# jipolanco/PencilArrays.jl

Measured on NVIDIA H100. Metric: transpose_GiB_per_s, higher is better.
Workload: dtype c128 (bytes; pure data movement)

## Files before the change

### pencilarrays.jl_b200/csrc/fft.cu

```cuda
#include <cuda_runtime.h>

#include <algorithm>
#include <cmath>
#include <map>
#include <mutex>
#include <tuple>
#include <type_traits>
#include <vector>

#ifndef PA_FFT_TWIDDLE_LOOKUPS
#define PA_FFT_TWIDDLE_LOOKUPS 1
#endif
#include "fft_core.hpp"
#include "flags.cuh"
#include "pa_internal.hpp"

namespace pa {

using pa_fft::cplx;
using pa_fft::cplx_t;

template <class T>
struct Vec2;
template <>
struct Vec2<double> {
  using type = double2;
};
template <>
struct Vec2<float> {
  using type = float2;
};
__device__ __forceinline__ double2 vec2(double x, double y) { return make_double2(x, y); }
__device__ __forceinline__ float2 vec2(float x, float y) { return make_float2(x, y); }

template <class T, int STRIDE = 1>
struct Twiddles {
  const typename Vec2<T>::type* tab;
  __device__ __forceinline__ cplx_t<T> operator()(int k) const {
    const typename Vec2<T>::type w = __ldg(tab + STRIDE * k);
    return cplx_t<T>{w.x, w.y};
  }
};

constexpr int FFT_MAXB = 8;
constexpr int FFT_MAXO = PA_MAX_DIMS - 2;
constexpr int FFT_THREADS = 256;
constexpr int fft_lines(int logL) { return logL >= 10 ? 4 : 8; }
constexpr int fft_lines_f32(int logL) { return logL >= 10 ? 8 : 16; }

struct FftBlock {
  const char* src;
  int y0, ey;
  long long ssy;
  long long ssx;
  long long so[FFT_MAXO];
};
struct FftParams {
  int nb;
  FftBlock blk[FFT_MAXB];
  char* dst;
  long long ex;
  long long dsx;
  int no;
  long long oe[FFT_MAXO], dso[FFT_MAXO];
  int L, logL, sign, pitch;
  int linear;
  const void* tw;
  unsigned tiles_x;
  const void* tw4;
  int sine;
};

template <class T>
struct SmLine {
  cplx_t<T>* p;
  __device__ __forceinline__ cplx_t<T> get(int i) const { return p[pa_fft::pad_index(i)]; }
  __device__ __forceinline__ void put(int i, cplx_t<T> v) { p[pa_fft::pad_index(i)] = v; }
};

template <int LOGM>
struct PassRadix {
  static constexpr int LOGR = (LOGM % 3 == 0) ? 3 : (LOGM % 3);
};

template <int LOGL, int LOGM, int C, class T, class Tw>
__device__ __forceinline__ void fft_passes(cplx_t<T>* sm, int pitch, int ncol, int sign, const Tw& tw) {
  if constexpr (LOGM > 0) {
    constexpr int LOGR = PassRadix<LOGM>::LOGR;
    constexpr int R = 1 << LOGR, L = 1 << LOGL, M = 1 << LOGM;
    constexpr int PER_LINE = L / R;
    constexpr int TOTAL = C * PER_LINE;
#pragma unroll
    for (int w0 = 0; w0 < TOTAL; w0 += FFT_THREADS) {
      const int w = w0 + (int)threadIdx.x;
      const int c = w / PER_LINE, u = w % PER_LINE;
      if (w < TOTAL && c < ncol) {
        SmLine<T> x{sm + c * pitch};
        pa_fft::butterfly<R>(x, u, L, M, sign, tw);
      }
    }
    __syncthreads();
    fft_passes<LOGL, LOGM - LOGR, C>(sm, pitch, ncol, sign, tw);
  }
}

template <int LOGL, int LOGM>
__device__ __forceinline__ int fft_pos(int k) {
  if constexpr (LOGM == 0) {
    return 0;
  } else {
    constexpr int LOGR = PassRadix<LOGM>::LOGR;
    return ((k & ((1 << LOGR) - 1)) << (LOGM - LOGR)) + fft_pos<LOGL, LOGM - LOGR>(k >> LOGR);
  }
}

template <int LOGL, class T>
__device__ __forceinline__ T out_real(const T* line, int i) {
  return line[2 * pa_fft::pad_index(fft_pos<LOGL, LOGL>(i >> 1)) + (i & 1)];
}

template <int C, class T>
__device__ __forceinline__ void gather_rows(const FftParams& p, const long long* so_off, long long x0,
                                            int c, int r, int ncol, cplx_t<T>* line) {
  using V = typename Vec2<T>::type;
  constexpr int RS = FFT_THREADS / C;
  constexpr int U = 8;
#pragma unroll
  for (int b = 0; b < FFT_MAXB; ++b) {
    if (b < p.nb) {
      const FftBlock& B = p.blk[b];
      const char* s = B.src + so_off[b] + (x0 + c) * B.ssx;
      const int ey = B.ey, y0 = B.y0;
      const long long ssy = B.ssy;
      for (int y = r; y < ey; y += U * RS) {
        V v[U];
#pragma unroll
        for (int k = 0; k < U; ++k) {
          const int yy = y + k * RS;
          if (c < ncol && yy < ey) v[k] = __ldcs(reinterpret_cast<const V*>(s + (long long)yy * ssy));
        }
#pragma unroll
        for (int k = 0; k < U; ++k) {
          const int yy = y + k * RS;
          if (c < ncol && yy < ey) line[pa_fft::pad_index(y0 + yy)] = cplx_t<T>{v[k].x, v[k].y};
        }
      }
    }
  }
}

enum class RealMap {
  rfft,
  dct2,
  dct3,
};

template <RealMap MAP, int LOGL, class T>
__device__ __forceinline__ void put_real(T* line, int n, T x, bool sine) {
  constexpr int L = 1 << LOGL, N = 2 * L;
  if constexpr (MAP == RealMap::rfft) {
    line[2 * pa_fft::pad_index(n >> 1) + (n & 1)] = x;
  } else if constexpr (MAP == RealMap::dct2) {
    const int i = (n & 1) ? N - 1 - (n >> 1) : (n >> 1);
    line[2 * pa_fft::pad_index(i >> 1) + (i & 1)] = ((n & 1) && sine) ? -x : x;
  } else {
    const int j = sine ? N - 1 - n : n;
    if (j <= L) line[2 * pa_fft::pad_index(j)] = x;
    if (j >= L) line[2 * pa_fft::pad_index(N - j) + 1] = x;
  }
}

template <int C, class T, class Put>
__device__ __forceinline__ void gather_real_rows(const FftParams& p, const long long* so_off, long long x0,
                                                 int c, int r, int ncol, const Put& put) {
  constexpr int RS = FFT_THREADS / C;
  constexpr int U = 8;
#pragma unroll
  for (int b = 0; b < FFT_MAXB; ++b) {
    if (b < p.nb) {
      const FftBlock& B = p.blk[b];
      const char* s = B.src + so_off[b] + (x0 + c) * B.ssx;
      const int ey = B.ey, y0 = B.y0;
      const long long ssy = B.ssy;
      for (int y = r; y < ey; y += U * RS) {
        T v[U];
#pragma unroll
        for (int k = 0; k < U; ++k) {
          const int yy = y + k * RS;
          if (c < ncol && yy < ey) v[k] = __ldcs(reinterpret_cast<const T*>(s + (long long)yy * ssy));
        }
#pragma unroll
        for (int k = 0; k < U; ++k) {
          const int yy = y + k * RS;
          if (c < ncol && yy < ey) put(y0 + yy, v[k]);
        }
      }
    }
  }
}

__device__ __forceinline__ long long cta_offsets(const FftParams& p, int C, long long* so_off,
                                                 long long* d_off) {
  unsigned long long bid = blockIdx.x;
  const long long x0 = (long long)(bid % p.tiles_x) * C;
  bid /= p.tiles_x;
#pragma unroll
  for (int b = 0; b < FFT_MAXB; ++b) so_off[b] = 0;
  *d_off = 0;
#pragma unroll 1
  for (int i = 0; i < p.no; ++i) {
    const long long k = (long long)(bid % (unsigned long long)p.oe[i]);
    bid /= (unsigned long long)p.oe[i];
    *d_off += k * p.dso[i];
#pragma unroll
    for (int b = 0; b < FFT_MAXB; ++b)
      if (b < p.nb) so_off[b] += k * p.blk[b].so[i];
  }
  return x0;
}

template <int LOGL, int C, class T>
struct FftCtaShape {
  static constexpr int RS = FFT_THREADS / C;
  static constexpr int LOGRS = (C == 16) ? 4 : (C == 8) ? 5 : 6;
  static_assert((1 << LOGRS) == RS, "rows per sweep");
  static constexpr int LOGR1 = (sizeof(T) == 8 && C == 4 && LOGL > LOGRS) ? (LOGL - LOGRS) : 0;
  static_assert(LOGR1 == 0 || LOGL - LOGR1 == LOGRS, "first-pass stride must equal the sweep");
  static_assert(LOGR1 <= 4, "the register first pass is at most radix 16");
};

template <int LOGL, int C, class T>
__device__ __forceinline__ void fft_cta_lines(const FftParams& p, const long long* so_off, long long x0,
                                              int ncol, cplx_t<T>* sm) {
  using cx = cplx_t<T>;
  using V = typename Vec2<T>::type;
  constexpr int L = 1 << LOGL;
  const int t = threadIdx.x;
  const int pitch = p.pitch;

  constexpr int RS = FftCtaShape<LOGL, C, T>::RS;
  constexpr int LOGR1 = FftCtaShape<LOGL, C, T>::LOGR1;
  const V* twp = reinterpret_cast<const V*>(p.tw);
  const Twiddles<T> tw{twp};
  {
    const int c = p.linear ? t / RS : t % C, r = p.linear ? t % RS : t / C;
    cx* line = sm + c * pitch;
    if constexpr (LOGR1 > 0) {
      constexpr int R1 = 1 << LOGR1;
      if (c < ncol) {
        V v[R1];
#pragma unroll
        for (int q = 0; q < R1; ++q) {
          const int y = r + q * RS;
          const char* s = nullptr;
#pragma unroll
          for (int b = 0; b < FFT_MAXB; ++b)
            if (b < p.nb && y >= p.blk[b].y0 && y < p.blk[b].y0 + p.blk[b].ey)
              s = p.blk[b].src + so_off[b] + (long long)(y - p.blk[b].y0) * p.blk[b].ssy +
                  (x0 + c) * p.blk[b].ssx;
          v[q] = __ldcs(reinterpret_cast<const V*>(s));
        }
        cx a[R1];
#pragma unroll
        for (int q = 0; q < R1; ++q) a[q] = cx{v[q].x, v[q].y};
        pa_fft::butterfly_regs<R1>(a, r, L, L, p.sign, tw);
#pragma unroll
        for (int q = 0; q < R1; ++q) line[pa_fft::pad_index(r + q * RS)] = a[q];
      }
    } else {
      gather_rows<C, T>(p, so_off, x0, c, r, ncol, line);
    }
  }
  __syncthreads();

  fft_passes<LOGL, LOGL - LOGR1, C>(sm, pitch, ncol, p.sign, tw);
}

template <int LOGL, int LOGR1>
__device__ __forceinline__ int fft_out_pos(int k) {
  return ((k & ((1 << LOGR1) - 1)) << (LOGL - LOGR1)) + fft_pos<LOGL, LOGL - LOGR1>(k >> LOGR1);
}

template <int LOGL, int C, class T>
__device__ __forceinline__ void unpack_fft_cta(const FftParams& p) {
  using cx = cplx_t<T>;
  using V = typename Vec2<T>::type;
  constexpr int L = 1 << LOGL;
  extern __shared__ __align__(16) unsigned char fft_smem[];
  cx* sm = reinterpret_cast<cx*>(fft_smem);
  const int t = threadIdx.x;
  long long so_off[FFT_MAXB], d_off;
  const long long x0 = cta_offsets(p, C, so_off, &d_off);
  const int ncol = (int)((p.ex - x0) < C ? (p.ex - x0) : C);
  const int pitch = p.pitch;
  constexpr int LOGR1 = FftCtaShape<LOGL, C, T>::LOGR1;

  fft_cta_lines<LOGL, C, T>(p, so_off, x0, ncol, sm);

  char* d = p.dst + x0 * p.dsx + d_off;
  for (int c = 0; c < ncol; ++c) {
    const cx* line = sm + c * pitch;
    V* out = reinterpret_cast<V*>(d + c * p.dsx);
#pragma unroll
    for (int k0 = 0; k0 < L; k0 += FFT_THREADS) {
      const int k = k0 + t;
      if (k < L) {
        const int pos = ((k & ((1 << LOGR1) - 1)) << (LOGL - LOGR1)) +
                        fft_pos<LOGL, LOGL - LOGR1>(k >> LOGR1);
        const cx v = line[pa_fft::pad_index(pos)];
        __stcs(out + k, vec2(v.x, v.y));
      }
    }
  }
}

template <int LOGL, int C, class T>
__global__ void __launch_bounds__(FFT_THREADS) k_unpack_fft(const __grid_constant__ FftParams p) {
  unpack_fft_cta<LOGL, C, T>(p);
}

struct FftGetParams {
  FftParams p;
  MultiFlags mf;
};
static_assert(sizeof(FftGetParams) <= 4096, "FftParams + MultiFlags must fit the kernel parameters");

template <int LOGL, int C, class T>
__global__ void __maxnreg__(128) k_get_fft(const __grid_constant__ FftGetParams gp) {
  const MultiFlags& mf = gp.mf;
  if (mf.ready.n > 0) {
    if ((int)threadIdx.x < mf.ready.n) {
      if (blockIdx.x < 8) flag_signal(mf.ready.remote[threadIdx.x], mf.ready.seq[threadIdx.x]);
      flag_wait(mf.ready.local[threadIdx.x], mf.ready.seq[threadIdx.x], mf.timeout_ns, mf.err);
    }
    __syncthreads();
  }
  unpack_fft_cta<LOGL, C, T>(gp.p);
  if (mf.done.n > 0) {
    __syncthreads();
    int last = 0;
    if (threadIdx.x == 0) {
      __threadfence_system();
      last = atomicAdd(mf.counter, 1u) == gridDim.x - 1;
      if (last) {
        *mf.counter = 0;
        __threadfence_system();
      }
    }
    if (__syncthreads_or(last) && (int)threadIdx.x < mf.done.n)
      flag_signal(mf.done.remote[threadIdx.x], mf.done.seq[threadIdx.x]);
  }
}

struct RfftParams {
  const char* src;
  char* dst;
  long long nlines;
  long long src_line, dst_line;
  int pitch;
  const void* tw;
};

template <int LOGL, int C, class T, class Out>
__device__ __forceinline__ void rfft_forward_tail(cplx_t<T>* sm, int pitch, int ncol, int t,
                                                  const typename Vec2<T>::type* twp, const Out& out) {
  using cx = cplx_t<T>;
  using V = typename Vec2<T>::type;
  constexpr int L = 1 << LOGL;
  constexpr int P = L / 2 + 1;
  const Twiddles<T> twN{twp};
  const Twiddles<T, 2> twL{twp};
  fft_passes<LOGL, LOGL, C>(sm, pitch, ncol, -1, twL);

#pragma unroll
  for (int w0 = 0; w0 < C * P; w0 += FFT_THREADS) {
    const int w = w0 + t, c = w / P, k = w % P;
    if (w < C * P && c < ncol) {
      const cx* line = sm + c * pitch;
      cx xk, xl;
      pa_fft::rfft_post_pair(line[pa_fft::pad_index(fft_pos<LOGL, LOGL>(k & (L - 1)))],
                             line[pa_fft::pad_index(fft_pos<LOGL, LOGL>((L - k) & (L - 1)))], twN(k),
                             &xk, &xl);
      V* o = reinterpret_cast<V*>(out(c));
      __stcs(o + k, vec2(xk.x, xk.y));
      if (k != L - k) __stcs(o + (L - k), vec2(xl.x, xl.y));
    }
  }
}

template <int LOGL, int C, bool UNROLL, class T>
__device__ __forceinline__ void brfft_pre(cplx_t<T>* sm, int pitch, int ncol, int t, const Twiddles<T>& twN) {
  using cx = cplx_t<T>;
  constexpr int L = 1 << LOGL;
  constexpr int P = L / 2 + 1;
  constexpr int TRIPS = (C * P + FFT_THREADS - 1) / FFT_THREADS;
#pragma unroll(UNROLL ? TRIPS : 1)
  for (int w0 = 0; w0 < C * P; w0 += FFT_THREADS) {
    const int w = w0 + t, c = w / P, k = w % P;
    if (w < C * P && c < ncol) {
      cx* line = sm + c * pitch;
      cx zk, zl;
      pa_fft::brfft_pre_pair(k, line[pa_fft::pad_index(k)], line[pa_fft::pad_index(L - k)], twN(k),
                             &zk, &zl);
      line[pa_fft::pad_index(k)] = zk;
      if (k > 0) line[pa_fft::pad_index(L - k)] = zl;
    }
  }
  __syncthreads();
}

template <int LOGL, int C, bool FWD, class T, class Src>
__device__ __forceinline__ void rfft_load(cplx_t<T>* sm, int pitch, int ncol, int t, const Src& src) {
  using cx = cplx_t<T>;
  using V = typename Vec2<T>::type;
  constexpr int L = 1 << LOGL;
  constexpr int RS = FFT_THREADS / C;
  constexpr int NIN = FWD ? L : L + 1;
  constexpr int U = (NIN + RS - 1) / RS;
  const int c = t / RS, r = t % RS;
  if (c < ncol) {
    const V* s = src(c);
    cx* line = sm + c * pitch;
    V v[U];
#pragma unroll
    for (int q = 0; q < U; ++q)
      if (r + q * RS < NIN) v[q] = __ldcs(s + r + q * RS);
#pragma unroll
    for (int q = 0; q < U; ++q)
      if (r + q * RS < NIN) line[pa_fft::pad_index(r + q * RS)] = cx{v[q].x, v[q].y};
  }
}

template <int LOGL, int C, bool FWD, class T>
__global__ void __launch_bounds__(FFT_THREADS) k_rfft(const __grid_constant__ RfftParams p) {
  using cx = cplx_t<T>;
  using V = typename Vec2<T>::type;
  constexpr int L = 1 << LOGL;
  extern __shared__ __align__(16) unsigned char fft_smem[];
  cx* sm = reinterpret_cast<cx*>(fft_smem);
  const int t = threadIdx.x;
  const long long l0 = (long long)blockIdx.x * C;
  const int ncol = (int)((p.nlines - l0) < C ? (p.nlines - l0) : C);
  const int pitch = p.pitch;
  const V* twp = reinterpret_cast<const V*>(p.tw);

  rfft_load<LOGL, C, FWD, T>(sm, pitch, ncol, t, [&p, l0](int c) {
    return reinterpret_cast<const V*>(p.src + (l0 + c) * p.src_line);
  });
  __syncthreads();

  if constexpr (FWD) {
    rfft_forward_tail<LOGL, C, T>(sm, pitch, ncol, t, twp,
                                  [&p, l0](int c) { return p.dst + (l0 + c) * p.dst_line; });
  } else {
    brfft_pre<LOGL, C, true, T>(sm, pitch, ncol, t, Twiddles<T>{twp});
    fft_passes<LOGL, LOGL, C>(sm, pitch, ncol, 1, Twiddles<T, 2>{twp});

#pragma unroll
    for (int w0 = 0; w0 < C * L; w0 += FFT_THREADS) {
      const int w = w0 + t, c = w >> LOGL, n = w & (L - 1);
      if (c < ncol) {
        const cx v = sm[c * pitch + pa_fft::pad_index(fft_pos<LOGL, LOGL>(n))];
        __stcs(reinterpret_cast<V*>(p.dst + (l0 + c) * p.dst_line) + n, vec2(v.x, v.y));
      }
    }
  }
}

template <int LOGL, int C, class T>
__global__ void __launch_bounds__(FFT_THREADS) k_unpack_brfft(const __grid_constant__ FftParams p) {
  using cx = cplx_t<T>;
  using V = typename Vec2<T>::type;
  constexpr int L = 1 << LOGL;
  constexpr int RS = FFT_THREADS / C;
  extern __shared__ __align__(16) unsigned char fft_smem[];
  cx* sm = reinterpret_cast<cx*>(fft_smem);
  const int t = threadIdx.x;
  long long so_off[FFT_MAXB], d_off;
  const long long x0 = cta_offsets(p, C, so_off, &d_off);
  const int ncol = (int)((p.ex - x0) < C ? (p.ex - x0) : C);
  const int pitch = p.pitch;
  const V* twp = reinterpret_cast<const V*>(p.tw);

  {
    const int c = p.linear ? t / RS : t % C, r = p.linear ? t % RS : t / C;
    gather_rows<C, T>(p, so_off, x0, c, r, ncol, sm + c * pitch);
  }
  __syncthreads();

  brfft_pre<LOGL, C, false, T>(sm, pitch, ncol, t, Twiddles<T>{twp});
  fft_passes<LOGL, LOGL, C>(sm, pitch, ncol, 1, Twiddles<T, 2>{twp});

  char* d = p.dst + x0 * p.dsx + d_off;
#pragma unroll
  for (int w0 = 0; w0 < C * L; w0 += FFT_THREADS) {
    const int w = w0 + t, c = w >> LOGL, n = w & (L - 1);
    if (c < ncol) {
      const cx v = sm[c * pitch + pa_fft::pad_index(fft_pos<LOGL, LOGL>(n))];
      __stcs(reinterpret_cast<V*>(d + c * p.dsx) + n, vec2(v.x, v.y));
    }
  }
}

struct R2rParams {
  const char* src;
  char* dst;
  long long nlines;
  long long line;
  int pitch;
  int sine;
  const void* tw;
  const void* tw4;
};

template <int LOGL, int C, class T>
__device__ __forceinline__ void r2r_pre(cplx_t<T>* sm, int pitch, int ncol, int t, const Twiddles<T>& twN,
                                        const Twiddles<T>& w4) {
  using cx = cplx_t<T>;
  constexpr int L = 1 << LOGL;
  constexpr int P = L / 2 + 1;
#pragma unroll
  for (int w0 = 0; w0 < C * P; w0 += FFT_THREADS) {
    const int w = w0 + t, c = w / P, k = w % P;
    if (w < C * P && c < ncol) {
      cx* line = sm + c * pitch;
      const cx vk = pa_fft::dct3_pre_pair(line[pa_fft::pad_index(k)], w4(k));
      const cx vl = pa_fft::dct3_pre_pair(line[pa_fft::pad_index(L - k)], w4(L - k));
      cx zk, zl;
      pa_fft::brfft_pre_pair(k, vk, vl, twN(k), &zk, &zl);
      line[pa_fft::pad_index(k)] = zk;
      if (k > 0) line[pa_fft::pad_index(L - k)] = zl;
    }
  }
  __syncthreads();
}

template <int LOGL, int C, bool FWD, class T, class Out>
__device__ __forceinline__ void r2r_tail(cplx_t<T>* sm, int pitch, int ncol, int t, bool sine,
                                         const typename Vec2<T>::type* twp,
                                         const typename Vec2<T>::type* tw4p, const Out& out) {
  using cx = cplx_t<T>;
  using V = typename Vec2<T>::type;
  constexpr int L = 1 << LOGL, N = 2 * L;
  constexpr int P = L / 2 + 1;
  const Twiddles<T> twN{twp};
  const Twiddles<T, 2> twL{twp};
  const Twiddles<T> w4{tw4p};

  if constexpr (!FWD) r2r_pre<LOGL, C, T>(sm, pitch, ncol, t, twN, w4);

  fft_passes<LOGL, LOGL, C>(sm, pitch, ncol, FWD ? -1 : 1, twL);

  if constexpr (FWD) {
#pragma unroll
    for (int w0 = 0; w0 < C * P; w0 += FFT_THREADS) {
      const int w = w0 + t, c = w / P, k = w % P;
      if (w < C * P && c < ncol) {
        const cx* line = sm + c * pitch;
        cx vk, vl;
        pa_fft::rfft_post_pair(line[pa_fft::pad_index(fft_pos<LOGL, LOGL>(k & (L - 1)))],
                               line[pa_fft::pad_index(fft_pos<LOGL, LOGL>((L - k) & (L - 1)))], twN(k),
                               &vk, &vl);
        T yk, ynk, yl, ynl;
        pa_fft::dct2_post_pair(vk, w4(k), &yk, &ynk);
        pa_fft::dct2_post_pair(vl, w4(L - k), &yl, &ynl);
        T* o = reinterpret_cast<T*>(out(c));
        auto put = [o, sine](int j, T y) { __stcs(o + (sine ? N - 1 - j : j), y); };
        put(k, yk);
        if (k > 0 && k < L / 2) put(N - k, ynk);
        if (k < L / 2) put(L - k, yl);
        if (k > 0) put(L + k, ynl);
      }
    }
  } else {
#pragma unroll
    for (int w0 = 0; w0 < C * L; w0 += FFT_THREADS) {
      const int w = w0 + t, c = w >> LOGL, m = w & (L - 1);
      if (c < ncol) {
        const T* line = reinterpret_cast<const T*>(sm + c * pitch);
        const int i = N - 1 - m;
        const T a = out_real<LOGL>(line, m);
        const T b = out_real<LOGL>(line, i);
        __stcs(reinterpret_cast<V*>(out(c)) + m, vec2(a, sine ? -b : b));
      }
    }
  }
}

template <int LOGL, int C, bool FWD, class T, class Src>
__device__ __forceinline__ void r2r_load(cplx_t<T>* sm, int pitch, int ncol, int t, bool sine,
                                         const Src& src) {
  using V = typename Vec2<T>::type;
  constexpr int L = 1 << LOGL, N = 2 * L;
  constexpr int RS = FFT_THREADS / C;
  constexpr int U = (L + RS - 1) / RS;
  const int c = t / RS, r = t % RS;
  if (c < ncol) {
    const V* s = src(c);
    T* line = reinterpret_cast<T*>(sm + c * pitch);
    V v[U];
#pragma unroll
    for (int q = 0; q < U; ++q)
      if (r + q * RS < L) v[q] = __ldcs(s + r + q * RS);
#pragma unroll
    for (int q = 0; q < U; ++q) {
      const int m = r + q * RS;
      if (m < L) {
        if constexpr (FWD) {
          line[2 * pa_fft::pad_index(m >> 1) + (m & 1)] = v[q].x;
          line[2 * pa_fft::pad_index((N - 1 - m) >> 1) + ((N - 1 - m) & 1)] = sine ? -v[q].y : v[q].y;
        } else {
          const int ja = sine ? N - 1 - 2 * m : 2 * m, jb = sine ? N - 2 - 2 * m : 2 * m + 1;
          if (ja <= L) line[2 * pa_fft::pad_index(ja)] = v[q].x;
          if (ja >= L) line[2 * pa_fft::pad_index(N - ja) + 1] = v[q].x;
          if (jb <= L) line[2 * pa_fft::pad_index(jb)] = v[q].y;
          if (jb >= L) line[2 * pa_fft::pad_index(N - jb) + 1] = v[q].y;
        }
      }
    }
    if (!FWD && r == 0) line[1] = T(0);
// ... 1103 lines not shown
```

Baseline: 1377.

## Fuse last radix-8 FFT pass into the store and generalize register first pass

Stops the shared-memory FFT passes before the final radix-8 stage and instead performs that butterfly in registers during the output store, writing strided results directly to global memory. The register-based first pass is generalized to other radices and line lengths, batching several butterfly groups of loads with a fast path for a single source block. It also adds a min-blocks launch bound for one configuration. The intent is to save one shared-memory round trip and one barrier, and to raise load-level parallelism, at the cost of more register pressure and less coalesced output stores.

Measured after the change: 1377, median of 6. About the same (-0.0%).

```diff
diff --git a/pencilarrays.jl_b200/csrc/fft.cu b/pencilarrays.jl_b200/csrc/fft.cu
--- a/pencilarrays.jl_b200/csrc/fft.cu
+++ b/pencilarrays.jl_b200/csrc/fft.cu
@@ -83,9 +83,9 @@
   static constexpr int LOGR = (LOGM % 3 == 0) ? 3 : (LOGM % 3);
 };
 
-template <int LOGL, int LOGM, int C, class T, class Tw>
+template <int LOGL, int LOGM, int C, int LOGSTOP = 0, class T, class Tw>
 __device__ __forceinline__ void fft_passes(cplx_t<T>* sm, int pitch, int ncol, int sign, const Tw& tw) {
-  if constexpr (LOGM > 0) {
+  if constexpr (LOGM > LOGSTOP) {
     constexpr int LOGR = PassRadix<LOGM>::LOGR;
     constexpr int R = 1 << LOGR, L = 1 << LOGL, M = 1 << LOGM;
     constexpr int PER_LINE = L / R;
@@ -100,7 +100,7 @@
       }
     }
     __syncthreads();
-    fft_passes<LOGL, LOGM - LOGR, C>(sm, pitch, ncol, sign, tw);
+    fft_passes<LOGL, LOGM - LOGR, C, LOGSTOP>(sm, pitch, ncol, sign, tw);
   }
 }
 
@@ -224,12 +224,13 @@
   static constexpr int RS = FFT_THREADS / C;
   static constexpr int LOGRS = (C == 16) ? 4 : (C == 8) ? 5 : 6;
   static_assert((1 << LOGRS) == RS, "rows per sweep");
-  static constexpr int LOGR1 = (sizeof(T) == 8 && C == 4 && LOGL > LOGRS) ? (LOGL - LOGRS) : 0;
-  static_assert(LOGR1 == 0 || LOGL - LOGR1 == LOGRS, "first-pass stride must equal the sweep");
+  static constexpr int LOGP = (sizeof(T) == 8 && C == 4 && LOGL == 10) ? 4 : PassRadix<LOGL>::LOGR;
+  static constexpr int LOGR1 = (LOGL - LOGP >= LOGRS) ? LOGP : 0;
+  static constexpr int NB = LOGR1 > 0 ? (1 << (LOGL - LOGR1 - LOGRS)) : 0;
   static_assert(LOGR1 <= 4, "the register first pass is at most radix 16");
 };
 
-template <int LOGL, int C, class T>
+template <int LOGL, int C, class T, int LOGSTOP = 0>
 __device__ __forceinline__ void fft_cta_lines(const FftParams& p, const long long* so_off, long long x0,
                                               int ncol, cplx_t<T>* sm) {
   using cx = cplx_t<T>;
@@ -246,26 +247,39 @@
     const int c = p.linear ? t / RS : t % C, r = p.linear ? t % RS : t / C;
     cx* line = sm + c * pitch;
     if constexpr (LOGR1 > 0) {
-      constexpr int R1 = 1 << LOGR1;
+      constexpr int R1 = 1 << LOGR1, Q1 = L >> LOGR1, NB = FftCtaShape<LOGL, C, T>::NB;
+      constexpr int G = R1 >= 8 ? 1 : (8 / R1 < NB ? 8 / R1 : NB);
       if (c < ncol) {
-        V v[R1];
-#pragma unroll
-        for (int q = 0; q < R1; ++q) {
-          const int y = r + q * RS;
-          const char* s = nullptr;
-#pragma unroll
-          for (int b = 0; b < FFT_MAXB; ++b)
-            if (b < p.nb && y >= p.blk[b].y0 && y < p.blk[b].y0 + p.blk[b].ey)
-              s = p.blk[b].src + so_off[b] + (long long)(y - p.blk[b].y0) * p.blk[b].ssy +
-                  (x0 + c) * p.blk[b].ssx;
-          v[q] = __ldcs(reinterpret_cast<const V*>(s));
+#pragma unroll 1
+        for (int i0 = 0; i0 < NB; i0 += G) {
+          V v[G * R1];
+#pragma unroll
+          for (int n = 0; n < G * R1; ++n) {
+            const int y = r + (i0 + n / R1) * RS + (n % R1) * Q1;
+            const char* s = nullptr;
+            if (p.nb == 1) {
+              s = p.blk[0].src + so_off[0] + (long long)(y - p.blk[0].y0) * p.blk[0].ssy +
+                  (x0 + c) * p.blk[0].ssx;
+            } else {
+#pragma unroll
+              for (int b = 0; b < FFT_MAXB; ++b)
+                if (b < p.nb && y >= p.blk[b].y0 && y < p.blk[b].y0 + p.blk[b].ey)
+                  s = p.blk[b].src + so_off[b] + (long long)(y - p.blk[b].y0) * p.blk[b].ssy +
+                      (x0 + c) * p.blk[b].ssx;
+            }
+            v[n] = __ldcs(reinterpret_cast<const V*>(s));
+          }
+#pragma unroll
+          for (int i = 0; i < G; ++i) {
+            const int j = r + (i0 + i) * RS;
+            cx a[R1];
+#pragma unroll
+            for (int q = 0; q < R1; ++q) a[q] = cx{v[i * R1 + q].x, v[i * R1 + q].y};
+            pa_fft::butterfly_regs<R1>(a, j, L, L, p.sign, tw);
+#pragma unroll
+            for (int q = 0; q < R1; ++q) line[pa_fft::pad_index(j + q * Q1)] = a[q];
+          }
         }
-        cx a[R1];
-#pragma unroll
-        for (int q = 0; q < R1; ++q) a[q] = cx{v[q].x, v[q].y};
-        pa_fft::butterfly_regs<R1>(a, r, L, L, p.sign, tw);
-#pragma unroll
-        for (int q = 0; q < R1; ++q) line[pa_fft::pad_index(r + q * RS)] = a[q];
       }
     } else {
       gather_rows<C, T>(p, so_off, x0, c, r, ncol, line);
@@ -273,7 +287,7 @@
   }
   __syncthreads();
 
-  fft_passes<LOGL, LOGL - LOGR1, C>(sm, pitch, ncol, p.sign, tw);
+  fft_passes<LOGL, LOGL - LOGR1, C, LOGSTOP>(sm, pitch, ncol, p.sign, tw);
 }
 
 template <int LOGL, int LOGR1>
@@ -295,27 +309,40 @@
   const int pitch = p.pitch;
   constexpr int LOGR1 = FftCtaShape<LOGL, C, T>::LOGR1;
 
-  fft_cta_lines<LOGL, C, T>(p, so_off, x0, ncol, sm);
-
+  fft_cta_lines<LOGL, C, T, 3>(p, so_off, x0, ncol, sm);
+
+  static_assert(LOGL >= 3 && LOGL - LOGR1 >= 3, "the last pass is radix 8");
+  constexpr int K = L / 8, TOTAL = C * K;
+  constexpr int LOGF = LOGR1 > 0 ? LOGR1 : PassRadix<LOGL>::LOGR;
+  constexpr int ROT = (LOGF < 3 && LOGL - 3 >= LOGF + 3) ? LOGF : 0;
+  const Twiddles<T> tw{reinterpret_cast<const V*>(p.tw)};
   char* d = p.dst + x0 * p.dsx + d_off;
-  for (int c = 0; c < ncol; ++c) {
-    const cx* line = sm + c * pitch;
-    V* out = reinterpret_cast<V*>(d + c * p.dsx);
-#pragma unroll
-    for (int k0 = 0; k0 < L; k0 += FFT_THREADS) {
-      const int k = k0 + t;
-      if (k < L) {
-        const int pos = ((k & ((1 << LOGR1) - 1)) << (LOGL - LOGR1)) +
-                        fft_pos<LOGL, LOGL - LOGR1>(k >> LOGR1);
-        const cx v = line[pa_fft::pad_index(pos)];
-        __stcs(out + k, vec2(v.x, v.y));
-      }
+#pragma unroll
+  for (int w0 = 0; w0 < TOTAL; w0 += FFT_THREADS) {
+    const int w = w0 + t;
+    const int c = w / K;
+    int kappa = w & (K - 1);
+    if constexpr (ROT > 0) {
+      const int kr = w & ((8 << ROT) - 1);
+      kappa = (kappa & ~((8 << ROT) - 1)) | ((kr & 7) << ROT) | (kr >> 3);
+    }
+    if (w < TOTAL && c < ncol) {
+      const SmLine<T> x{sm + c * pitch};
+      const int base = fft_out_pos<LOGL, LOGR1>(kappa);
+      cx a[8];
+#pragma unroll
+      for (int q = 0; q < 8; ++q) a[q] = x.get(base + q);
+      pa_fft::butterfly_regs<8>(a, 0, L, 8, p.sign, tw);
+      V* out = reinterpret_cast<V*>(d + c * p.dsx);
+#pragma unroll
+      for (int s = 0; s < 8; ++s) __stcs(out + kappa + s * K, vec2(a[s].x, a[s].y));
     }
   }
 }
 
 template <int LOGL, int C, class T>
-__global__ void __launch_bounds__(FFT_THREADS) k_unpack_fft(const __grid_constant__ FftParams p) {
+__global__ void __launch_bounds__(FFT_THREADS, (sizeof(T) == 8 && C == 8) ? 3 : 0)
+    k_unpack_fft(const __grid_constant__ FftParams p) {
   unpack_fft_cta<LOGL, C, T>(p);
 }
 
```
